# giesselmann/STRique

Measured on AMD Instinct MI355X. Metric: reads/s for STRique 'count' on 50 kb r9.4 signals, higher is better.
Workload: dtype f32

## Files before the change

strique_amd/csrc/screen_kernels.hip:

```cpp
#include "strq_opt.h"
#include <hip/hip_runtime.h>
#include <stdint.h>
#include <stdlib.h>
#include <cmath>
#include "screen_kernels.h"
#include "screen_lds_layout.h"
#include "screen_levels_layout.h"

namespace strq {

namespace {

constexpr int R = STRQ_SCREEN_R, S = STRQ_SCREEN_S, SEG = STRQ_SCREEN_SEG;
constexpr int G = 2, C = 3;
static_assert(R == 14 && S == 6, "class expansion below is written for 14 rows per lane, 6 samples per class");

__device__ __forceinline__ int dpp_shr1(int v, int fill)
{
    return __builtin_amdgcn_update_dpp(fill, v, 0x138, 0xF, 0xF, false);
}
__device__ __forceinline__ int dpp_shr1_open(int v)
{
    return __builtin_amdgcn_mov_dpp(v, 0x138, 0xF, 0xF, true);
}
// ... 181 lines not shown
                    lc.lo2[c] = lo * 2; lc.hi2[c] = (lo + w1) * 2;
                    lc.off[c] = (off - lo) * 2;
                } else {
                    lc.lo2[c] = 0; lc.hi2[c] = 0; lc.off[c] = zero_idx * 2;
                }
            }
            pm[0] = 0;
#pragma unroll
            for (int x = 1; x < 3; ++x) {
                const uint64_t b = __ballot(phase >= S - x * G);
                const uint32_t lo = __builtin_amdgcn_readfirstlane((int)(uint32_t)b), hi = __builtin_amdgcn_readfirstlane((int)(uint32_t)(b >> 32));
                pm[x] = ((uint64_t)hi << 32) | lo;
            }
        }
        const int lM = (tk.m - 1) / R;
        Screen f{ldsb, lc, pm, lane, tk.n, sp.hh};
        {
#pragma unroll
            for (int r = 0; r < R; ++r) f.T[r] = STRQ_SCREEN_BIAS;
            f.SbotA = STRQ_SCREEN_BIAS; f.upS = STRQ_SCREEN_BIAS;
            f.potB = STRQ_SCREEN_BIAS - 2 * lane * sp.hh;
            f.cmax = STRQ_SCREEN_BIAS;
        }
        const int nsteps = (tk.n + 1) / 2 + 63;
        int qcur = load_chunk(tk, 0, lane);
        f.prime(qcur);
        for (int t0s = 0; t0s < nsteps; t0s += 64) {
            const int qnext = load_chunk(tk, t0s / 64 + 1, lane);
            const bool full = (t0s >= 63) && (2 * (t0s + 64) <= tk.n);
            const int send = nsteps - t0s < 64 ? nsteps - t0s : 64;
            if (full) {
                for (int s = 0; s < 63; ++s) f.template step<false>(t0s + s + 1, qcur, s + 1);
                f.template step<false>(t0s + 64, qnext, 0);
            } else {
                for (int s = 0; s < send; ++s) {
                    const int qsrc = s == 63 ? qnext : qcur, snext = (s + 1) & 63;
                    f.template step<true>(t0s + s + 1, qsrc, snext);
                }
            }
            const int cm = __builtin_amdgcn_readlane(f.cmax, lM) - STRQ_SCREEN_BIAS;
            if (lane == 0) tk.out[t0s / 64] = cm;
            f.cmax = STRQ_SCREEN_BIAS;
            qcur = qnext;
        }
    }
}

namespace {

constexpr int CPL = STRQ_SCREEN2_CPL, LPF = STRQ_SCREEN2_LPF, LB = STRQ_SCREEN2_LANE_B;

struct Lane2Const { int lo2[CPL], hi2[CPL], off[CPL]; };

template <int RPC, int CMG, int LAYOUT>
struct Screen2 {
    static constexpr int R2 = RPC * CPL;
    static constexpr bool LEVELS = LAYOUT == STRQ_SCREEN_LDS_LEVELS;
    static_assert(CMG == 1 || CMG == 2 || CMG == 4, "groups must divide the 64 steps of a chunk");
    const char* lds;
    const Lane2Const& lc;
    const uint64_t top_mask;
    const int lane, n, hh;
    int T[R2], SbotA, upS, potB, cmax;
    int gpot, gmax;
    int qq;
    int scA[CPL], scB[CPL];

    template <bool HI>
    __device__ __forceinline__ int column(int qpair) const
    {
        if constexpr (LEVELS) return HI ? mad3_hi16(qpair, lc.off[0]) : mad3_lo16(qpair, lc.off[0]);
        else return HI ? (int)((unsigned)qpair >> 16) : (qpair & 0xffff);
    }
    __device__ __forceinline__ int score(int q2, int c) const
    {
        if constexpr (LEVELS) return *reinterpret_cast<const uint8_t*>(lds + q2 + screen_levels::class_offset(c));
        else return *reinterpret_cast<const uint16_t*>(lds + med3i(q2, lc.lo2[c], lc.hi2[c]) + lc.off[c]);
    }
    __device__ __forceinline__ void prime(int qcur)
    {
        qq = __builtin_amdgcn_update_dpp(__builtin_amdgcn_readlane(qcur, 0), 0, 0x138, 0xF, 0xF, false);
        const int qa = column<false>(qq), qb = column<true>(qq);
#pragma unroll
        for (int c = 0; c < CPL; ++c) { scA[c] = score(qa, c); scB[c] = score(qb, c); }
    }

    template <bool PRED>
    __device__ __forceinline__ void step(int t, int qsrc, int snext, bool gfirst = true, bool glast = true)
    {
        const int qn = __builtin_amdgcn_update_dpp(__builtin_amdgcn_readlane(qsrc, snext), qq, 0x138, 0xF, 0xF, false);
        const int qa = column<false>(qn), qb = column<true>(qn);
        const int potA = add_uniform(potB, hh), potBn = add_uniform(potA, hh);
        const int upA = sel_mask(dpp_shr1_open(SbotA), potA, top_mask);
        const int upB = sel_mask(dpp_shr1_open(T[R2 - 1]), potBn, top_mask);
        constexpr bool GROUPED = !PRED && CMG > 1;
        if (GROUPED && gfirst) gpot = potA;
        bool act = true, okB = true;
        if constexpr (PRED) { const int jB = 2 * (t - lane), jA = jB - 1; act = (jA >= 1) && (jA <= n); okB = jB <= n; }
        int ta_prev = upA, ta_prev2 = upS;
        int tb_prev2 = upB;
#pragma unroll
        for (int c = 0; c < CPL; ++c) {
            if (act) {
#pragma unroll
                for (int r = RPC * c; r < RPC * c + RPC; ++r) {
                    const int diagA = r == 0 ? upS : T[r - 1];
                    const int ta = max3i(diagA + scA[c], T[r], ta_prev);
                    if (r > 0) {
                        const int tb = max3i(ta_prev2 + scB[(r - 1) / RPC], ta_prev, tb_prev2);
                        T[r - 1] = tb; tb_prev2 = tb;
                    }
                    ta_prev2 = ta_prev; ta_prev = ta;
                }
                if (c == CPL - 1) {
                    const int tb = max3i(ta_prev2 + scB[c], ta_prev, tb_prev2);
                    T[R2 - 1] = tb;
                    SbotA = ta_prev;
                    upS = upB;
                    if constexpr (GROUPED) {
                        if (glast) { const int d = tb - gpot; gmax = d > gmax ? d : gmax; }
                    } else {
                        const int cA = ta_prev - potA + STRQ_SCREEN_BIAS, cB = okB ? tb - potBn + STRQ_SCREEN_BIAS : cA;
                        cmax = max3i(cmax, cA, cB);
                    }
                }
            }
            scA[c] = score(qa, c);
            if (c > 0) scB[c - 1] = score(qb, c - 1);
            if (c == CPL - 1) scB[c] = score(qb, c);
        }
        potB = potBn;
        qq = qn;
    }
};

template <int SHIFT, bool LEVELS>
__device__ __forceinline__ int load_chunk2(const Screen2Task& tk, int chunk, int lane, int lvl0, int lvl1)
{
    const int idx = (chunk * 64 + lane) * 2;
    int a = 0, b = 0;
    if (idx < tk.n) a = tk.levels[idx];
    if (idx + 1 < tk.n) b = tk.levels[idx + 1];
    if constexpr (LEVELS) return screen_levels::scaled_level(a, lvl0, lvl1) | (screen_levels::scaled_level(b, lvl0, lvl1) << 16);
    else return (a << SHIFT) | (b << (SHIFT + 16));
}

template <int RPC, int CMG, int LAYOUT, int SEGW>
__device__ __forceinline__ void screen2_body(const Screen2Task* __restrict__ tasks, int n_groups, int* __restrict__ queue, const ScreenParams& sp, int lds_rows)
{
    constexpr int R2 = RPC * CPL, MERGE = S / RPC;
    constexpr bool LANES = LAYOUT == STRQ_SCREEN_LDS_LANES, LEVELS = LAYOUT == STRQ_SCREEN_LDS_LEVELS;
    constexpr int QSHIFT = LANES ? screen_lanes::ROW_SHIFT : 1;
    constexpr int UNIT = LEVELS ? MERGE : 1;
    static_assert(!LEVELS || (MERGE == screen_levels::MERGE && SEGW == screen_levels::SEG && CPL == screen_levels::CPL), "the level image is the coarse screen's");
    static_assert((SEGW & (SEGW - 1)) == 0, "the prologue deals rows to waves by a mask");
    static_assert(CPL == screen_lanes::CPL, "screen_lds_layout.h stacks the lane's five classes");
    extern __shared__ uint32_t lds_all[];
    __shared__ int next_group;
    const int lane = threadIdx.x & 63, wave = threadIdx.x >> 6;
    const char* ldsb = reinterpret_cast<const char*>(lds_all);
    const int f = lane >= LB ? 1 : 0, lf = lane - f * LB;
    for (;;) {
        __syncthreads();
        if (threadIdx.x == 0) next_group = atomicAdd(queue, 1);
        __syncthreads();
        const int gi = __builtin_amdgcn_readfirstlane(next_group);
        if (gi >= n_groups) break;
        const Screen2Task& t0 = tasks[(size_t)gi * SEGW];
        const int ksc = LEVELS ? sp.byte_sc : sp.sc;
        const int khh = LEVELS ? sp.hh * ksc / sp.sc : sp.hh, kcadd = LEVELS ? khh + sp.v * ksc / sp.sc : sp.cadd;
        const float scf = (float)ksc;
        Lane2Const lc;
        [[maybe_unused]] int lvl0 = 0, lvl1 = 0;
        if constexpr (LEVELS) {
            lvl0 = screen_levels::range_lo(t0.lvl); lvl1 = screen_levels::range_hi(t0.lvl);
            uint32_t desc[CPL];
            int nc = 0;
#pragma unroll
            for (int c = 0; c < CPL; ++c) {
                const int k = lf * CPL + c;
                const bool in = lf < LPF && k < t0.k[f];
                desc[c] = in ? (uint32_t)t0.band_lo[f][k] : 0u;
                nc += in ? 1 : 0;
            }
            char* dst = reinterpret_cast<char*>(lds_all) + screen_levels::slot(lane);
            const float* src = t0.table[f];
            const int rows = lvl1 - lvl0 + 1 < lds_rows ? lvl1 - lvl0 + 1 : lds_rows;
            for (int r = wave; r < rows; r += SEGW) {
                int e[CPL];
#pragma unroll
                for (int c = 0; c < CPL; ++c) {
                    e[c] = 0;
                    if (c < nc) {
                        const int v = ceil_scaled(src[screen_levels::desc_off(desc[c]) + screen_levels::band_index(desc[c], lvl0 + r)], scf) + kcadd;
                        e[c] = v < 255 ? v : 255;
                    }
                }
                char* row = dst + r * screen_levels::ROW_BYTES;
                *reinterpret_cast<uint16_t*>(row + screen_levels::class_offset(0)) = (uint16_t)(e[0] | (e[1] << 8));
                *reinterpret_cast<uint16_t*>(row + screen_levels::class_offset(2)) = (uint16_t)(e[2] | (e[3] << 8));
                *reinterpret_cast<uint16_t*>(row + screen_levels::class_offset(4)) = (uint16_t)e[4];
            }
#pragma unroll
            for (int c = 0; c < CPL; ++c) { lc.lo2[c] = 0; lc.hi2[c] = 0; lc.off[c] = screen_levels::slot(lane); }
        }
        if constexpr (LANES) {
            uint32_t desc[CPL];
            int nc = 0, rowbase[CPL];
#pragma unroll
            for (int c = 0; c < CPL; ++c) {
                const int k = lf * CPL + c;
                const bool in = lf < LPF && k < t0.k[f];
                desc[c] = in ? (uint32_t)t0.band_lo[f][k] : 0u;
                nc += in ? 1 : 0;
            }
            screen_lanes::row_bases(desc, nc, rowbase);
            char* dst = reinterpret_cast<char*>(lds_all);
            if (wave == 0) *reinterpret_cast<uint16_t*>(dst + screen_lanes::slot(lane)) = 0;
#pragma unroll
            for (int c = 0; c < CPL; ++c) {
                const screen_lanes::ClassAddr a = c < nc ? screen_lanes::class_addr(lane, rowbase[c], desc[c]) : screen_lanes::padding_addr(lane);
                lc.lo2[c] = a.lo2; lc.hi2[c] = a.hi2; lc.off[c] = a.off;
                if (c < nc) {
                    const float* src = t0.table[f] + screen_lanes::desc_off(desc[c]);
                    const int w1 = screen_lanes::desc_w1(desc[c]);
                    for (int i = (wave - rowbase[c]) & (SEGW - 1); i <= w1; i += SEGW)
                        if (rowbase[c] + i < lds_rows)
                            *reinterpret_cast<uint16_t*>(dst + screen_lanes::entry_address(lane, rowbase[c], i)) = (uint16_t)(MERGE * (ceil_scaled(src[i], scf) + sp.cadd));
                }
            }
        }
        [[maybe_unused]] int base[2], zero_idx[2];
        base[0] = 0; zero_idx[0] = (t0.tsize[0] + 1) & ~1;
        base[1] = zero_idx[0] + 2; zero_idx[1] = base[1] + ((t0.tsize[1] + 1) & ~1);
        if constexpr (!LANES && !LEVELS) {
            uint16_t* dst = reinterpret_cast<uint16_t*>(lds_all);
#pragma unroll
            for (int ff = 0; ff < 2; ++ff) {
                for (int i = threadIdx.x; i < t0.tsize[ff]; i += 64 * SEGW) dst[base[ff] + i] = (uint16_t)(MERGE * (ceil_scaled(t0.table[ff][i], scf) + sp.cadd));
                if (threadIdx.x == 0) { dst[zero_idx[ff]] = 0; dst[zero_idx[ff] + 1] = 0; }
            }
        }
        __syncthreads();
        const Screen2Task& tk = tasks[(size_t)gi * SEGW + wave];
        if (tk.n <= 0) continue;

        if constexpr (!LANES && !LEVELS) {
#pragma unroll
            for (int c = 0; c < CPL; ++c) {
                const int k = lf * CPL + c;
                if (lf < LPF && k < tk.k[f]) {
                    const uint32_t d = (uint32_t)tk.band_lo[f][k];
                    const int lo = (int)(d & 255u), w1 = (int)((d >> 8) & 255u), off = (int)(d >> 16);
                    lc.lo2[c] = lo * 2; lc.hi2[c] = (lo + w1) * 2;
                    lc.off[c] = (base[f] + off - lo) * 2;
                } else {
                    lc.lo2[c] = 0; lc.hi2[c] = 0; lc.off[c] = zero_idx[f] * 2;
                }
            }
        }
        const uint64_t top_mask = 1ull | (1ull << LB);
        const int lMa = (tk.k[0] - 1) / CPL, lMb = LB + (tk.k[1] - 1) / CPL;
        const int hh = khh / UNIT;
        Screen2<RPC, CMG, LAYOUT> s2{ldsb, lc, top_mask, lane, tk.n, hh};
        {
#pragma unroll
            for (int r = 0; r < R2; ++r) s2.T[r] = STRQ_SCREEN_BIAS;
            s2.SbotA = STRQ_SCREEN_BIAS; s2.upS = STRQ_SCREEN_BIAS;
            s2.potB = STRQ_SCREEN_BIAS - 2 * lane * hh;
            s2.cmax = STRQ_SCREEN_BIAS; s2.gpot = 0; s2.gmax = 0;
        }
        const int nsteps = (tk.n + 1) / 2 + 63;
        int qcur = load_chunk2<QSHIFT, LEVELS>(tk, 0, lane, lvl0, lvl1);
        s2.prime(qcur);
        for (int t0s = 0; t0s < nsteps; t0s += 64) {
            const int qnext = load_chunk2<QSHIFT, LEVELS>(tk, t0s / 64 + 1, lane, lvl0, lvl1);
            const bool full = (t0s >= 63) && (2 * (t0s + 64) <= tk.n);
            const int send = nsteps - t0s < 64 ? nsteps - t0s : 64;
            if (full) {
                constexpr int U = CMG > 2 ? CMG : 2;
                s2.gmax = 0;
#pragma unroll 1
                for (int s = 0; s < 64 - U; s += U) {
#pragma unroll
                    for (int u = 0; u < U; ++u) s2.template step<false>(0, qcur, s + u + 1, u % CMG == 0, u % CMG == CMG - 1);
                }
#pragma unroll
                for (int u = 0; u < U - 1; ++u) s2.template step<false>(0, qcur, 64 - U + u + 1, u % CMG == 0, u % CMG == CMG - 1);
                s2.template step<false>(0, qnext, 0, CMG == 1, true);
                if constexpr (CMG > 1) s2.cmax = s2.gmax + STRQ_SCREEN_BIAS;
            } else {
                for (int s = 0; s < send; ++s) {
                    const int qsrc = s == 63 ? qnext : qcur, snext = (s + 1) & 63;
                    s2.template step<true>(t0s + s + 1, qsrc, snext);
                }
            }
            const int cma = __builtin_amdgcn_readlane(s2.cmax, lMa) - STRQ_SCREEN_BIAS;
            const int cmb = __builtin_amdgcn_readlane(s2.cmax, lMb) - STRQ_SCREEN_BIAS;
            if (lane == 0) {
                if constexpr (LEVELS) {
                    tk.out[0][t0s / 64] = (int)(((long long)cma * UNIT * sp.sc + ksc - 1) / ksc);
                    tk.out[1][t0s / 64] = (int)(((long long)cmb * UNIT * sp.sc + ksc - 1) / ksc);
                } else { tk.out[0][t0s / 64] = cma; tk.out[1][t0s / 64] = cmb; }
            }
            s2.cmax = STRQ_SCREEN_BIAS;
            qcur = qnext;
        }
    }
}

}

size_t screen2_lds_bytes(int tsize_a, int tsize_b)
{
    return (size_t)(((tsize_a + 1) & ~1) + 2 + ((tsize_b + 1) & ~1) + 2) * 2;
}

int screen2_lanes_rows(int need_a, int need_b) { return screen_lanes::rows_bound(need_a, need_b); }
bool screen2_lanes_fit(int rows) { return screen_lanes::fits(rows); }
size_t screen2_lanes_lds_bytes(int rows) { return screen_lanes::bytes(rows); }

#ifndef STRQ_SCREEN3_CMG
#define STRQ_SCREEN3_CMG 2
#endif
#define STRQ_SCREEN2_ATTR_SEG(WPE_, SEG_) __attribute__((amdgpu_flat_work_group_size(64 * SEG_, 64 * SEG_), amdgpu_waves_per_eu(WPE_, WPE_)))
#define STRQ_SCREEN2_ATTR(WPE_) STRQ_SCREEN2_ATTR_SEG(WPE_, STRQ_SCREEN_SEG)
#define STRQ_SCREEN2_ARGS const Screen2Task* __restrict__ tasks, int n_groups, int* __restrict__ queue, ScreenParams sp, int lds_rows
__global__ void STRQ_SCREEN2_ATTR_SEG(6, STRQ_SCREEN_SEG_LEVELS) align_screen3_kernel(STRQ_SCREEN2_ARGS) { screen2_body<2, STRQ_SCREEN3_CMG, STRQ_SCREEN_LDS_LEVELS, STRQ_SCREEN_SEG_LEVELS>(tasks, n_groups, queue, sp, lds_rows); }
__global__ void STRQ_SCREEN2_ATTR(6) align_screen3_lanes_kernel(STRQ_SCREEN2_ARGS) { screen2_body<2, STRQ_SCREEN3_CMG, STRQ_SCREEN_LDS_LANES, STRQ_SCREEN_SEG>(tasks, n_groups, queue, sp, lds_rows); }
__global__ void STRQ_SCREEN2_ATTR(4) align_screen1_kernel(STRQ_SCREEN2_ARGS) { screen2_body<6, 1, STRQ_SCREEN_LDS_LANES, STRQ_SCREEN_SEG>(tasks, n_groups, queue, sp, lds_rows); }
__global__ void STRQ_SCREEN2_ATTR(6) align_screen3_rows_kernel(STRQ_SCREEN2_ARGS) { screen2_body<2, STRQ_SCREEN3_CMG, STRQ_SCREEN_LDS_ROWS, STRQ_SCREEN_SEG>(tasks, n_groups, queue, sp, lds_rows); }
__global__ void STRQ_SCREEN2_ATTR(4) align_screen1_rows_kernel(STRQ_SCREEN2_ARGS) { screen2_body<6, 1, STRQ_SCREEN_LDS_ROWS, STRQ_SCREEN_SEG>(tasks, n_groups, queue, sp, lds_rows); }
#undef STRQ_SCREEN2_ARGS

__global__ void __launch_bounds__(256)
screen_windows_kernel(const ScreenTask* __restrict__ tasks, int n_groups, ScreenParams sp,
                      const int32_t* __restrict__ bound_scaled, ScreenWindows* __restrict__ out,
                      const int32_t* __restrict__ list, const int32_t* __restrict__ theta_list)
{
    const int lane = threadIdx.x & 63;
    const int idx = blockIdx.x * (blockDim.x >> 6) + (threadIdx.x >> 6);
    if (idx >= n_groups) return;
    const int g = list ? list[idx] : idx;
    const int SEG = sp.seg;
    const ScreenTask* tg = tasks + (size_t)g * SEG;
    const int m = tg[0].m, lM = tg[0].lane_last;
    const int shift = -m * sp.v;
    int vmax = 0;
    for (int w = 0; w < SEG; ++w) {
        if (tg[w].n <= 0) continue;
        for (int c = lane; c < tg[w].n_chunks; c += 64) { const int v = tg[w].out[c]; vmax = v > vmax ? v : vmax; }
    }
#pragma unroll
    for (int d = 32; d >= 1; d >>= 1) { const int o = __shfl_xor(vmax, d, 64); vmax = o > vmax ? o : vmax; }
    ScreenWindows r;
    r.n_win = 0; r.n_cand = 0;
    for (int k = 0; k < STRQ_SCREEN_MAX_WINDOWS; ++k) { r.lo[k] = 0; r.hi[k] = 0; }
    const int drop = (sp.margin > 0 ? sp.margin : m) + 2 * sp.slack;
    int theta = theta_list ? theta_list[idx] : vmax - drop;
    if (!theta_list && sp.max_cand > 0) {
        auto count_at = [&](int t) {
            int n = 0;
            for (int w = 0; w < SEG; ++w) {
                if (tg[w].n <= 0) continue;
                for (int c = lane; c < tg[w].n_chunks; c += 64) n += tg[w].out[c] >= t;
            }
#pragma unroll
            for (int d = 32; d >= 1; d >>= 1) n += __shfl_xor(n, d, 64);
            return n;
        };
        if (count_at(theta) > sp.max_cand) {
            int lo = theta, hi = vmax;
            while (hi - lo > 1) {
                const int mid = lo + (hi - lo) / 2;
                if (count_at(mid) > sp.max_cand) lo = mid; else hi = mid;
            }
            theta = hi;
        }
    }
    r.upper_bound = (float)(vmax + shift + sp.slack) / (float)sp.sc;
    auto scan = [&](int th, bool store) -> int {
        int nw = 0, last_hi = -(1 << 30), ncand = 0;
        for (int w = 0; w < SEG; ++w) {
            if (tg[w].n <= 0) continue;
            for (int c0 = 0; c0 < tg[w].n_chunks; c0 += 64) {
                const int c1 = c0 + lane;
                const bool cand = c1 < tg[w].n_chunks && tg[w].out[c1] >= th;
                uint64_t mask = __ballot(cand);
                while (mask) {
                    const int bit = __builtin_ctzll(mask); mask &= mask - 1;
                    const int c = c0 + bit;
                    ++ncand;
                    int lo = 128 * c - 2 * lM + 1, hi = 128 * c - 2 * lM + 128;
                    if (lo < 1) lo = 1;
                    if (hi > tg[w].n) hi = tg[w].n;
                    if (hi < lo) continue;
                    lo += tg[w].col_off; hi += tg[w].col_off;
                    if (nw > 0 && lo <= last_hi + sp.merge_gap) {
                        if (hi > last_hi) last_hi = hi;
                        if (store) {
                            const int k = nw <= STRQ_SCREEN_MAX_WINDOWS ? nw - 1 : STRQ_SCREEN_MAX_WINDOWS - 1;
                            if (hi > r.hi[k]) r.hi[k] = hi;
                            if (lo < r.lo[k]) r.lo[k] = lo;
                        }
                    } else {
                        ++nw; last_hi = hi;
                        if (store) {
                            if (nw <= STRQ_SCREEN_MAX_WINDOWS) { r.lo[nw - 1] = lo; r.hi[nw - 1] = hi; }
                            else if (hi > r.hi[STRQ_SCREEN_MAX_WINDOWS - 1]) r.hi[STRQ_SCREEN_MAX_WINDOWS - 1] = hi;
                        }
                    }
                }
            }
        }
        if (store) r.n_cand = ncand;
        return nw;
    };
    if (!theta_list && sp.max_cand > 0 && scan(theta, false) > STRQ_SCREEN_MAX_WINDOWS) {
        int lo = theta, hi = vmax;
        while (hi - lo > 1) {
            const int mid = lo + (hi - lo) / 2;
            if (scan(mid, false) > STRQ_SCREEN_MAX_WINDOWS) lo = mid; else hi = mid;
        }
        theta = hi;
    }
    {
        const double lb = (double)(theta + shift + sp.slack) / (double)sp.sc;
        float lbf = (float)lb;
        if ((double)lbf < lb) {
            int32_t bits = __float_as_int(lbf);
            bits = lbf > 0.0f ? bits + 1 : (lbf < 0.0f ? bits - 1 : 1);
            lbf = __int_as_float(bits);
        }
        r.lower_bound = lbf;
    }
    const bool ok = theta + shift > 0 && theta + shift > bound_scaled[g];
    if (ok) {
        int nw = scan(theta, true);
        if (nw > STRQ_SCREEN_MAX_WINDOWS) nw = STRQ_SCREEN_MAX_WINDOWS;
        for (int a = 1; a < nw; ++a)
            for (int b = a; b > 0 && r.lo[b] < r.lo[b - 1]; --b) {
                const int tl = r.lo[b], th = r.hi[b]; r.lo[b] = r.lo[b - 1]; r.hi[b] = r.hi[b - 1]; r.lo[b - 1] = tl; r.hi[b - 1] = th;
            }
        int kept = nw > 0 ? 1 : 0;
        for (int a = 1; a < nw; ++a) {
            if (r.lo[a] <= r.hi[kept - 1] + 1) { if (r.hi[a] > r.hi[kept - 1]) r.hi[kept - 1] = r.hi[a]; }
            else { r.lo[kept] = r.lo[a]; r.hi[kept] = r.hi[a]; ++kept; }
        }
        for (int a = kept; a < STRQ_SCREEN_MAX_WINDOWS; ++a) { r.lo[a] = 0; r.hi[a] = 0; }
        r.n_win = kept;
    }
    if (lane == 0) out[idx] = r;
}

int screen_plan(const AlignParams& p, int samples, int max_n, ScreenParams* sp)
{
    if (strq::opt("STRQ_NO_SCREEN")) return 0;
    if (samples != S) return 0;
    if (!(p.open_h == p.ext_h && p.open_v == p.ext_v)) return 0;
    if (!(p.dist_min >= 0.0f) || !(p.ext_h < 0.0f) || !(p.ext_v < 0.0f) || !(p.dist_offset > 0.0f) || !(p.dist_min <= p.dist_offset)) return 0;
    for (int sc = 1024; sc >= 16; sc >>= 1) {
        const double hh = -(double)p.ext_h * sc, v = -(double)p.ext_v * sc, smax = std::ceil((double)p.dist_offset * sc);
        if (hh != (double)(long)hh || v != (double)(long)v) continue;
        if (hh < 1 || smax + v + hh > 65000.0) continue;
        const double top = 64.0 * R * (smax + v) + ((double)max_n + 256.0) * hh + smax + v + hh + (double)STRQ_SCREEN_BIAS;
        if (top > 2.0e9) continue;
        sp->sc = sc; sp->hh = (int)hh; sp->v = (int)v; sp->cadd = (int)(hh + v);
        {
            const double rows = 64.0 * R, maxval = rows * (double)p.dist_offset;
            double p2 = 1.0; while (p2 < maxval) p2 *= 2.0;
            const double adds = rows * (1.0 + (double)p.dist_offset / -(double)p.ext_h);
            const double e = adds * p2 / 16777216.0;
            if (!(e < 1.0e4)) continue;
            sp->slack = ((int)std::ceil(e) + 1) * sc;
        }
        sp->merge_gap = 3072; sp->margin = 0; sp->max_cand = 0; sp->seg = STRQ_SCREEN_SEG; sp->byte_sc = 0;
        return 1;
    }
    return 0;
}

int screen2_plan(const AlignParams& p, int samples, int max_n, int merge, ScreenParams* sp)
{
    if (merge != 1 && merge != 3) return 0;
    if (!screen_plan(p, samples, max_n, sp)) return 0;
    while (sp->sc >= 16) {
        const double smax = std::ceil((double)p.dist_offset * sp->sc);
        if ((double)merge * (smax + sp->cadd) <= 65000.0) return 1;
        if ((sp->hh & 1) || (sp->v & 1)) return 0;
        sp->slack = (sp->slack / sp->sc) * (sp->sc / 2);
        sp->sc /= 2; sp->hh /= 2; sp->v /= 2; sp->cadd = sp->hh + sp->v;
    }
    return 0;
}

int screen2_levels_plan(const AlignParams& p, int samples, int max_n, int merge, ScreenParams* sp)
{
    if (merge != screen_levels::MERGE) return 0;
    if (!screen2_plan(p, samples, max_n, merge, sp)) return 0;
    const int bsc = screen_levels::byte_scale((double)p.ext_h, (double)p.ext_v, (double)p.dist_offset);
    if (bsc <= 0) return 0;
    const double hhb = -(double)p.ext_h * bsc;
    if ((double)(max_n + 256) * hhb / screen_levels::MERGE + 64.0 * CPL * 2 * 255.0 + (double)STRQ_SCREEN_BIAS > 2.0e9) return 0;
    sp->byte_sc = bsc; sp->seg = STRQ_SCREEN_SEG_LEVELS;
    return 1;
}

ScreenParams screen2_byte_frame(const ScreenParams& sp)
{
    ScreenParams b = sp;
    const int bsc = sp.byte_sc;
    b.hh = (int)((long long)sp.hh * bsc / sp.sc); b.v = (int)((long long)sp.v * bsc / sp.sc); b.cadd = b.hh + b.v;
    b.slack = sp.slack / sp.sc * bsc; b.sc = bsc; b.seg = STRQ_SCREEN_SEG; b.byte_sc = 0;
    return b;
}

uint32_t screen2_levels_range(uint32_t lvl_a, uint32_t lvl_b) { return screen_levels::join_ranges(lvl_a, lvl_b); }
int screen2_levels_rows(uint32_t range) { return screen_levels::rows_of(range); }
bool screen2_levels_fit(int rows) { return screen_levels::fits(rows); }
size_t screen2_levels_lds_bytes(int rows) { return screen_levels::bytes(rows); }

int launch_screen2(hipStream_t stream, const Screen2Task* tasks, int n_groups, int* queue, const ScreenParams& sp,
                   size_t lds_bytes, int groups_per_cu, int n_cu, int merge, int layout, int rows)
{
    if (n_groups <= 0) return 0;
    if (merge != 3 && merge != 1) return 2;
    const bool lanes = layout == STRQ_SCREEN_LDS_LANES, levels = layout == STRQ_SCREEN_LDS_LEVELS;
    if (!lanes && !levels && layout != STRQ_SCREEN_LDS_ROWS) return 2;
    if (lanes && (!screen_lanes::fits(rows) || lds_bytes < screen_lanes::bytes(rows))) return 2;
    if (levels) {
        if (merge != screen_levels::MERGE || !screen_levels::fits(rows) || lds_bytes < screen_levels::bytes(rows) || sp.seg != STRQ_SCREEN_SEG_LEVELS || sp.byte_sc <= 0) return 2;
        const ScreenParams b = screen2_byte_frame(sp);
        if (b.hh < screen_levels::MERGE || b.hh % screen_levels::MERGE != 0 || b.cadd > 255 || (long long)b.hh * sp.sc != (long long)sp.hh * b.sc) return 2;
    }
    if (!levels && sp.seg != SEG) return 2;
    auto kern = merge == 3 ? (levels ? align_screen3_kernel : lanes ? align_screen3_lanes_kernel : align_screen3_rows_kernel) : (lanes ? align_screen1_kernel : align_screen1_rows_kernel);
    if (merge == 1 && groups_per_cu > 4) groups_per_cu = 4;
    if (groups_per_cu > 6) groups_per_cu = 6;
    (void)hipFuncSetAttribute((const void*)kern, hipFuncAttributeMaxDynamicSharedMemorySize, (int)lds_bytes);
    hipLaunchKernelGGL(kern, dim3(groups_per_cu * n_cu), dim3(64 * sp.seg), lds_bytes, stream, tasks, n_groups, queue, sp, lanes || levels ? rows : 0);
    return hipGetLastError() == hipSuccess ? 0 : 1;
}

int launch_screen(hipStream_t stream, const ScreenTask* tasks, int n_groups, int* queue, const ScreenParams& sp,
                  size_t lds_bytes, int tables_per_cu, int n_cu)
{
    if (n_groups <= 0) return 0;
    (void)hipFuncSetAttribute((const void*)align_screen_kernel, hipFuncAttributeMaxDynamicSharedMemorySize, (int)lds_bytes);
    hipLaunchKernelGGL(align_screen_kernel, dim3(tables_per_cu * n_cu), dim3(64 * SEG), lds_bytes, stream, tasks, n_groups, queue, sp);
    return hipGetLastError() == hipSuccess ? 0 : 1;
}

int launch_screen_windows(hipStream_t stream, const ScreenTask* tasks, int n_groups, const ScreenParams& sp,
                          const int32_t* bound_scaled, ScreenWindows* out, const int32_t* list, const int32_t* theta_list)
{
    if (n_groups <= 0) return 0;
    hipLaunchKernelGGL(screen_windows_kernel, dim3((n_groups + 3) / 4), dim3(256), 0, stream, tasks, n_groups, sp, bound_scaled, out, list, theta_list);
    return hipGetLastError() == hipSuccess ? 0 : 1;
}

}
```

strique_amd/csrc/screen_levels_layout.h:

```cpp
#pragma once
#include <stddef.h>
#include <stdint.h>

#if defined(__HIPCC__) || defined(__CUDACC__)
#define STRQ_LEVELS_HD __host__ __device__ __forceinline__
#else
#define STRQ_LEVELS_HD inline
#endif

namespace strq {
namespace screen_levels {

constexpr int SUB_BYTES = 128;
constexpr int SUBS = 3;
constexpr int ROW_BYTES = SUBS * SUB_BYTES;
constexpr int Q_SHIFT = 7;
constexpr int CPL = 5;
constexpr int MERGE = 3;
constexpr int SEG = 8;
static_assert(SUB_BYTES == 1 << Q_SHIFT && 255 * SUB_BYTES < 65536, "a scaled level has to fit the 16-bit half of the level pair");

constexpr int MAX_ROWS = 183;
constexpr size_t MAX_BYTES = (size_t)MAX_ROWS * ROW_BYTES;

STRQ_LEVELS_HD int desc_lo(uint32_t d) { return (int)(d & 255u); }
STRQ_LEVELS_HD int desc_w1(uint32_t d) { return (int)((d >> 8) & 255u); }
STRQ_LEVELS_HD int desc_off(uint32_t d) { return (int)(d >> 16); }

STRQ_LEVELS_HD uint32_t pack_range(int lvl0, int lvl1) { return (uint32_t)lvl0 | ((uint32_t)lvl1 << 8); }
STRQ_LEVELS_HD int range_lo(uint32_t r) { return (int)(r & 255u); }
STRQ_LEVELS_HD int range_hi(uint32_t r) { return (int)((r >> 8) & 255u); }
STRQ_LEVELS_HD uint32_t join_ranges(uint32_t a, uint32_t b)
{
    const int lo = range_lo(a) < range_lo(b) ? range_lo(a) : range_lo(b), hi = range_hi(a) > range_hi(b) ? range_hi(a) : range_hi(b);
    return pack_range(lo, hi < lo ? lo : hi);
}
STRQ_LEVELS_HD int rows_of(uint32_t r) { return range_hi(r) - range_lo(r) + 1; }

STRQ_LEVELS_HD int slot(int lane) { return (lane & 31) * 4 + (lane >> 5) * 2; }
STRQ_LEVELS_HD int class_offset(int c) { return (c >> 1) * SUB_BYTES + (c & 1); }

STRQ_LEVELS_HD int scaled_level(int level, int lvl0, int lvl1)
{
    const int l = level < lvl0 ? lvl0 : (level > lvl1 ? lvl1 : level);
    return (l - lvl0) << Q_SHIFT;
}
STRQ_LEVELS_HD int column_address(int scaled, int lane) { return scaled * SUBS + slot(lane); }
STRQ_LEVELS_HD int address(int lane, int c, int level, int lvl0, int lvl1) { return column_address(scaled_level(level, lvl0, lvl1), lane) + class_offset(c); }
STRQ_LEVELS_HD int band_index(uint32_t desc, int level)
{
    const int lo = desc_lo(desc), w1 = desc_w1(desc);
    return level < lo ? 0 : (level > lo + w1 ? w1 : level - lo);
}

STRQ_LEVELS_HD size_t bytes(int rows) { return (size_t)rows * ROW_BYTES; }
STRQ_LEVELS_HD bool fits(int rows) { return rows >= 1 && rows <= MAX_ROWS; }

inline int byte_scale(double ext_h, double ext_v, double dist_offset)
{
    for (int sc = 255; sc >= 1; --sc) {
        const double hh = -ext_h * sc, v = -ext_v * sc;
        if (hh != (double)(long)hh || v != (double)(long)v || hh < MERGE) continue;
        if ((long)hh % MERGE != 0) continue;
        const double top = dist_offset * sc;
        const long smax = (long)top + ((double)(long)top < top ? 1 : 0);
        if ((double)smax + hh + v > 255.0) continue;
        return sc;
    }
    return 0;
}

}
}
```

strique_amd/csrc/strq_align_api.hip:

```cpp
#include <hip/hip_runtime.h>
#include <algorithm>
#include <cmath>
#include <climits>
#include <cstring>
#include <cstdlib>
#include <time.h>
#include <unistd.h>
#include <map>
#include <mutex>
#include <string>
#include <tuple>
#include <numeric>
#include <vector>
#include "../../include/strique_hip.h"
#include "strq_ctx.h"
#include "align_kernels.h"
#include "lut_kernels.h"
#include "align_generic.h"

using namespace strq;

#define STRQ_DBG(...) do { if (strq::opt("STRQ_DEBUG")) { fprintf(stderr, "[strq] " __VA_ARGS__); fprintf(stderr, "\n"); fflush(stderr); } } while (0)

namespace strq {
// ... 391 lines not shown
        const uint32_t lvl = F == 2 ? screen2_levels_range((uint32_t)p.info[p.J0[a[0]]].lvl, (uint32_t)p.info[p.J0[a[1]]].lvl) : 0u;
        if (F == 2) j.levels_rows = std::max(j.levels_rows, screen2_levels_rows(lvl));
        for (int f = 0; f < F; ++f)
            j.bound[(size_t)g * F + f] = used <= 1 ? INT32_MIN / 2 : (ov_s >= ov_worst ? 0 : (int32_t)std::ceil((double)align_segment_min_score(p.c->ap, in.m[a[f]], ov_s) * sp.sc));
        for (int w = 0; w < SSEG; ++w) {
            Screen2Task t; std::memset(&t, 0, sizeof(t));
            t.levels = in.d_levels + in.read_off[in.read[a[0]]] + pc[w].col_off;
            t.n = pc[w].n; t.col_off = pc[w].col_off; t.lvl = lvl;
            t.n_chunks = pc[w].n > 0 ? (align_num_steps(pc[w].n) + 63) / 64 : 0;
            for (int f = 0; f < F; ++f) {
                const LutJob& job = p.jobs[p.J0[a[f]]];
                t.table[f] = job.table; t.band_lo[f] = job.band_lo; t.tsize[f] = p.info[p.J0[a[f]]].total; t.k[f] = in.k[a[f]];
                ScreenTask v; std::memset(&v, 0, sizeof(v));
                v.n = pc[w].n; v.m = in.m[a[f]]; v.k = in.k[a[f]]; v.col_off = pc[w].col_off; v.n_chunks = t.n_chunks;
                if (F == 2) v.lane_last = f * STRQ_SCREEN2_LANE_B + (in.k[a[f]] - 1) / STRQ_SCREEN2_CPL;
                else { v.levels = t.levels; v.table = t.table[0]; v.band_lo = t.band_lo[0]; v.tsize = t.tsize[0]; v.lane_last = (v.m - 1) / STRQ_SCREEN_R; }
                j.out_off[((size_t)g * F + f) * SSEG + w] = j.out_words; j.out_words += (size_t)t.n_chunks;
                j.views[((size_t)g * F + f) * SSEG + w] = v;
            }
            if (pc[w].n > 0) j.steps += align_num_steps(pc[w].n);
            if (F == 2) j.t2[(size_t)g * SSEG + w] = t;
        }
    }
}

static int run_screen(CorePlan& p, ScreenJob& j, const ScreenParams& sp, const ScreenRules& r)
{
    const int SSEG = sp.seg;
    strq_ctx* c = p.c; const AlignCoreIn& in = p.in;
    hipStream_t st = p.st;
    const int nv = (int)j.al.size();
    int layout = 0, image_rows = 0;
    if (j.flanks == 2) {
        const char* e = strq::opt("STRQ_SCREEN_LDS");
        layout = STRQ_SCREEN_LDS_ROWS;
        if (j.layout == STRQ_SCREEN_LDS_LEVELS) { layout = STRQ_SCREEN_LDS_LEVELS; image_rows = j.levels_rows; j.lds_bytes = screen2_levels_lds_bytes(image_rows); }
        else if (!(e && std::strcmp(e, "rows") == 0) && screen2_lanes_fit(j.lanes_rows)) { layout = STRQ_SCREEN_LDS_LANES; image_rows = j.lanes_rows; j.lds_bytes = screen2_lanes_lds_bytes(image_rows); }
    }
    if (j.lds_bytes > 160 * 1024 - 64) { c->err = r.lds_err; return STRQ_ERR_UNSUPPORTED; }
    const int groups = std::max(1, std::min(r.groups_per_cu, (int)((160 * 1024 - 64) / j.lds_bytes)));
    auto aligned = [](size_t bytes) { return (bytes + 255) & ~(size_t)255; };
    const size_t t2_bytes = aligned(j.t2.size() * sizeof(Screen2Task)), task_bytes = aligned(j.views.size() * sizeof(ScreenTask));
    const size_t bound_bytes = aligned((size_t)nv * 4), win_bytes = aligned((size_t)nv * sizeof(ScreenWindows));
    STRQ_HIP(c, c->screen.reserve(t2_bytes + task_bytes + bound_bytes + win_bytes + j.out_words * 4 + 256));
    char* base = c->screen.as<char>();
    Screen2Task* d_t2 = reinterpret_cast<Screen2Task*>(base);
    ScreenTask* d_st = reinterpret_cast<ScreenTask*>(base + t2_bytes);
    int32_t* d_bound = reinterpret_cast<int32_t*>(base + t2_bytes + task_bytes);
    ScreenWindows* d_win = reinterpret_cast<ScreenWindows*>(base + t2_bytes + task_bytes + bound_bytes);
    int32_t* d_out = reinterpret_cast<int32_t*>(base + t2_bytes + task_bytes + bound_bytes + win_bytes);
    for (size_t x = 0; x < j.views.size(); ++x) j.views[x].out = d_out + j.out_off[x];
    if (j.flanks == 2)
        for (int v = 0; v < nv; ++v) for (int w = 0; w < SSEG; ++w) j.t2[(size_t)(v / 2) * SSEG + w].out[v % 2] = j.views[(size_t)v * SSEG + w].out;
    if (j.flanks == 2) STRQ_HIP(c, hipMemcpyAsync(d_t2, j.t2.data(), j.t2.size() * sizeof(Screen2Task), hipMemcpyHostToDevice, st));
    STRQ_HIP(c, hipMemcpyAsync(d_st, j.views.data(), j.views.size() * sizeof(ScreenTask), hipMemcpyHostToDevice, st));
    STRQ_HIP(c, hipMemcpyAsync(d_bound, j.bound.data(), (size_t)nv * 4, hipMemcpyHostToDevice, st));
    STRQ_HIP(c, hipEventRecord(c->ev[5], st));
    int* queue = c->queue.as<int>() + STRQ_QUEUE_FIRST - 1;
    if (j.flanks == 2) {
        if (launch_screen2(st, d_t2, nv / 2, queue, sp, j.lds_bytes, groups, c->n_cu, r.merge, layout, image_rows)) { c->err = "coarse screen launch failed"; return STRQ_ERR_DEVICE; }
    } else {
        if (launch_screen(st, d_st, nv, queue, sp, j.lds_bytes, groups, c->n_cu)) { c->err = "screen launch failed"; return STRQ_ERR_DEVICE; }
    }
    STRQ_HIP(c, hipEventRecord(c->ev[6], st));
    if (launch_screen_windows(st, d_st, nv, sp, d_bound, d_win)) { c->err = "screen windows launch failed"; return STRQ_ERR_DEVICE; }
    std::vector<ScreenWindows> hw((size_t)nv);
    STRQ_HIP(c, hipMemcpyAsync(hw.data(), d_win, hw.size() * sizeof(ScreenWindows), hipMemcpyDeviceToHost, st));
    STRQ_HIP(c, hipStreamSynchronize(st));
    c->screen_ran = true; c->screen_mode_last = r.merge > 1 ? 2 : 1; c->coarse_merge_last = r.merge;
    c->screen_lds_last = layout; c->screen_byte_sc_last = layout == STRQ_SCREEN_LDS_LEVELS ? sp.byte_sc : 0;
    if (const char* path = strq::opt("STRQ_SCREEN_DUMP")) {
        std::vector<int32_t> ho(j.out_words);
        STRQ_HIP(c, hipMemcpy(ho.data(), d_out, j.out_words * 4, hipMemcpyDeviceToHost));
        if (FILE* fp = fopen(path, "wb")) {
            const int32_t hdr[8] = {nv, sp.sc, sp.hh, sp.v, j.flanks, SSEG, sp.slack, r.merge};
            fwrite(hdr, 4, 8, fp);
            for (int v = 0; v < nv; ++v) {
                const int32_t gh[4] = {j.al[v], j.al[v], j.bound[v], j.views[(size_t)v * SSEG].lane_last};
                fwrite(gh, 4, 4, fp);
                for (int w = 0; w < SSEG; ++w) {
                    const ScreenTask& t = j.views[(size_t)v * SSEG + w];
                    const int32_t th[4] = {t.col_off, t.n, t.m, t.n_chunks};
                    fwrite(th, 4, 4, fp);
                    fwrite(ho.data() + (t.out - d_out), 4, (size_t)t.n_chunks, fp);
                }
                fwrite(&hw[(size_t)v], sizeof(ScreenWindows), 1, fp);
            }
            fclose(fp);
        }
    }
    if (const char* e = strq::opt("STRQ_SCREEN_TEST_RAISE")) {
        const float up = (float)atof(e);
        for (auto& w : hw) w.lower_bound += up;
    }
    int windowed = 0, heavy = 0, below_bound = 0; double cols = 0, all = 0;
    for (int v = 0; v < nv; ++v) {
        const int al = j.al[v];
        const ScreenWindows& w = hw[(size_t)v];
        c->screen_stats[1] += 1; c->screen_stats[7] += w.n_cand;
        double mine = in.n[al];
        if (w.n_win > 0) {
            p.wins[al] = w; c->screen_stats[2] += 1; ++windowed; mine = 0;
            for (int k = 0; k < w.n_win; ++k) { c->screen_stats[4] += w.hi[k] - w.lo[k] + 1; mine += w.hi[k] - w.lo[k] + 1 + 4096; }
        } else {
            c->screen_stats[3] += 1;
            if (w.n_cand == 0) { ++below_bound; if (r.below_bound_free) mine = 0; }
        }
        all += in.n[al]; cols += mine; heavy += mine > 4 * 32768.0;
    }
    if (r.count_untaken) c->screen_stats[3] += p.nb - nv;
    c->screen_stats[5] += j.steps; c->screen_stats[6] = sp.sc;
    if (j.flanks == 2) {
        p.screen2_ran = true;
        p.d_st2 = d_st; p.d_bound2 = d_bound; p.sp2 = sp;
        for (int v = 0; v < nv; ++v) p.g2_of[j.al[v]] = v;
        p.coarse_cols = cols; p.coarse_all = all;
    }
    if (r.judge && nv >= 64) {
        if (below_bound * 10 > nv && !p.ov_fixed) c->score_fracs.clear();
        else if (windowed < 0.9 * (nv - (p.ov_fixed ? 0 : below_bound)) || cols > r.max_cols * all || (long)heavy * 100 > 2L * nv) pause_after_fail(*r.pause, *r.fail);
        else *r.fail = 0;
    }
    STRQ_DBG("screen (%d flanks per wave, merge %d, LDS layout %d, %d image rows, %d pieces): %d alignments, scale %d, margin %.0f, %d groups per CU, LDS %zu bytes: %d with windows (%d below the cold-start bound), %.2f %% of the columns, %d heavy -> pause %d",
             j.flanks, r.merge, layout, image_rows, SSEG, nv, sp.sc, (double)sp.margin / sp.sc, groups, j.lds_bytes, windowed, below_bound, 100.0 * cols / std::max(1.0, all), heavy, *r.pause);
    return STRQ_OK;
}

static int screen_two_flank(CorePlan& p, int merge, int max_n)
{
    strq_ctx* c = p.c; const AlignCoreIn& in = p.in;
    const int nb = p.nb;
    ScreenParams sp;
    if (!screen2_plan(c->ap, p.S, max_n, merge, &sp)) return STRQ_OK;
    const bool fine_rules = merge == 1;
    int min_n = fine_rules ? 65536 : 28672, groups = 6;
    if (const char* e = strq::opt("STRQ_SCREEN_MIN_N")) min_n = atoi(e);
    if (const char* e = strq::opt("STRQ_SCREEN2_GROUPS")) { const int v = atoi(e); if (v >= 1 && v <= 8) groups = v; }
    std::map<int, std::vector<int>> by_read;
    for (int i = 0; i < nb; ++i)
        if (in.NS[i] == 1 && p.NJ[i] == 1 && in.n[i] >= min_n && screen2_flank_ok(in.m[i], in.k[i])) by_read[in.read[i]].push_back(i);
    std::vector<std::pair<int, int>> pairs;
    for (auto& kv : by_read) {
        const std::vector<int>& v = kv.second;
        if (v.size() == 2) { pairs.emplace_back(v[0], v[1]); continue; }
        for (size_t x = 0; x + 1 < v.size(); ++x)
            if (!(v[x] & 1) && v[x + 1] == v[x] + 1) { pairs.emplace_back(v[x], v[x + 1]); ++x; }
    }
    std::stable_sort(pairs.begin(), pairs.end(), [&](const std::pair<int, int>& x, const std::pair<int, int>& y) { return in.n[x.first] > in.n[y.first]; });
    const int ngr = (int)pairs.size();
    if (ngr == 0 || 2 * ngr < (nb * 9) / 10) return STRQ_OK;
    bool levels = false;
    if (merge == 3) {
        const char* e = strq::opt("STRQ_SCREEN_LDS");
        ScreenParams spb;
        if (screen2_levels_plan(c->ap, p.S, max_n, merge, &spb)) {
            levels = !e || std::strcmp(e, "levels") == 0;
            for (size_t x = 0; levels && x < pairs.size(); ++x)
                levels = screen2_levels_fit(screen2_levels_rows(screen2_levels_range((uint32_t)p.info[p.J0[pairs[x].first]].lvl, (uint32_t)p.info[p.J0[pairs[x].second]].lvl)));
            if (levels && !e) {
                double extra = 0, all = 0; long used = 0;
                for (const auto& pr : pairs) {
                    const int m_big = std::max(in.m[pr.first], in.m[pr.second]);
                    const int ov_s = overlap_for(p, m_big, align_segment_overlap(c->ap, m_big), 16);
                    Piece pc[STRQ_SCREEN_SEG_MAX];
                    const int u8 = cut(in.n[pr.first], STRQ_SCREEN_SEG_LEVELS, ov_s, pc), u4 = cut(in.n[pr.first], STRQ_SCREEN_SEG, ov_s, pc);
                    extra += (double)(u8 - u4) * ov_s; all += in.n[pr.first]; used += u8;
                }
                levels = extra <= 0.10 * all && used * 10 >= 9L * STRQ_SCREEN_SEG_LEVELS * (long)pairs.size();
            }
            if (levels) sp = spb;
            else if (strq::opt("STRQ_SCREEN2_BYTE_SCALE")) sp = screen2_byte_frame(spb);
        }
    }
    sp.margin = (int32_t)std::lround((double)c->coarse_margin * (merge == 3 ? 1.3 : 1.0) * sp.sc);
    if (const char* e = strq::opt("STRQ_SCREEN2_MARGIN")) sp.margin = (int32_t)std::lround(atof(e) * sp.sc);
    sp.max_cand = 8;
    if (const char* e = strq::opt("STRQ_SCREEN2_MAX_CAND")) sp.max_cand = atoi(e);
    if (fine_rules) { sp.margin = 0; sp.max_cand = 0; }
    ScreenJob j;
    j.flanks = 2;
    for (const auto& pr : pairs) { j.al.push_back(pr.first); j.al.push_back(pr.second); }
    j.layout = levels ? STRQ_SCREEN_LDS_LEVELS : 0;
    screen_tasks(p, sp, j);
    ScreenRules r;
    r.merge = merge; r.groups_per_cu = groups;
    r.lds_err = "score tables do not fit LDS (coarse screen)";
    r.below_bound_free = !p.ov_fixed; r.count_untaken = true;
    if (fine_rules) { r.judge = !p.scr_forced; r.max_cols = 0.15; r.pause = &c->screen_pause; r.fail = &c->screen_fail; }
    else { r.judge = !p.mode_coarse && !p.scr_forced; r.max_cols = 0.30; r.pause = &c->coarse_pause; r.fail = &c->coarse_fail; }
    return run_screen(p, j, sp, r);
}

static int screen_one_flank(CorePlan& p, const ScreenParams& sp)
{
    strq_ctx* c = p.c; const AlignCoreIn& in = p.in;
    int min_n = 65536;
    if (const char* e = strq::opt("STRQ_SCREEN_MIN_N")) min_n = atoi(e);
    std::vector<int> sel;
    for (int i = 0; i < p.nb; ++i)
        if (in.NS[i] == 1 && p.NJ[i] == 1 && in.n[i] >= min_n && screen_flank_ok(in.m[i]) && in.k[i] * p.S == in.m[i]) sel.push_back(i);
    std::stable_sort(sel.begin(), sel.end(), [&](int x, int y) { return in.n[x] > in.n[y]; });
    if (sel.empty()) return STRQ_OK;
    ScreenJob j;
    j.al = sel;
    screen_tasks(p, sp, j);
    ScreenRules r;
    r.merge = 0; r.groups_per_cu = 6;
    r.lds_err = "score table does not fit LDS (screen)";
    r.below_bound_free = false; r.count_untaken = false;
    r.judge = true; r.max_cols = 0.10; r.pause = &c->screen_pause; r.fail = &c->screen_fail;
    return run_screen(p, j, sp, r);
}

static int run_screens(CorePlan& p)
{
    strq_ctx* c = p.c; const AlignCoreIn& in = p.in;
    const int nb = p.nb;
    p.wins.resize(nb);
    c->screen_ran = false;
    STRQ_HIP(c, hipEventRecord(c->ev[2], p.st));
    int max_n = 0;
    for (int i = 0; i < nb; ++i) max_n = std::max(max_n, in.n[i]);
    c->screen_mode_last = 0;
    const int coarse_merge = 3;
    p.g2_of.assign(nb, -1);
    for (int attempt = 0; attempt < 2 && !p.screen2_ran; ++attempt) {
        int merge = coarse_merge;
        if (attempt == 0) {
            if (!p.collapsed || p.mode_fine || strq::opt("STRQ_NO_SCREEN")) continue;
            if (c->coarse_pause > 0 && !p.mode_coarse && !p.scr_forced) { --c->coarse_pause; continue; }
        } else {
            if (!p.collapsed || strq::opt("STRQ_NO_SCREEN") || (c->screen_pause > 0 && !p.scr_forced)) continue;
            merge = 1;
        }
        const int rc = screen_two_flank(p, merge, max_n);
        if (rc) return rc;
    }
    if (p.screen2_ran) return STRQ_OK;
    if (p.collapsed && c->screen_pause > 0 && !p.scr_forced) {
        --c->screen_pause; c->screen_stats[3] += nb;
        return STRQ_OK;
    }
    ScreenParams sp;
    if (p.collapsed && screen_plan(c->ap, p.S, max_n, &sp)) return screen_one_flank(p, sp);
    return STRQ_OK;
}

static int plan_launches(CorePlan& p)
{
    strq_ctx* c = p.c; const AlignCoreIn& in = p.in; AlignCoreOut& out = p.out;
    const int nb = p.nb;
    std::vector<ScreenWindows>& wins = p.wins;
    static const double rate[5][2] = {{0, 0}, {1.017, 0.941}, {0.79, 0.862}, {0.85, 0.85}, {0.69, 0.80}};
    p.packed.assign(nb, 0); p.overlap.assign(nb, 0); p.segs_of.assign(nb, 1);
    std::vector<char> segmentable(nb, 0);
    const bool force_pack = strq::opt("STRQ_PACK") != nullptr;
    int class_count[5] = {0, 0, 0, 0, 0};
    for (int i = 0; i < nb; ++i) {
        segmentable[i] = p.collapsed && in.NS[i] == 1;
        p.overlap[i] = segmentable[i] ? align_segment_overlap(c->ap, in.m[i]) : 0;
        const bool can_pack = p.allow_pack && in.NS[i] == 1 && p.info[p.J0[i]].packed && p.info[p.J0[i]].n_hard == 0;
        int best_s = 1, best_p = can_pack ? 1 : 0;
        if (segmentable[i]) {
            const double l = overlap_for(p, in.m[i], p.overlap[i]);
            double best_cost = 0;
            for (int sgs : {1, 2, 3, 4}) {
                if (p.seg_want ? sgs != p.seg_want : sgs == 3) continue;
                if (sgs > 1 && !p.seg_want && (l <= 0 || in.n[i] < (sgs + 1) * l)) continue;
                for (int pk = 0; pk < 2; ++pk) {
                    if ((pk && !can_pack) || (force_pack && can_pack && !pk)) continue;
                    const double cost = (in.n[i] + (sgs - 1) * l) * rate[sgs][pk];
                    if (best_cost == 0 || cost < best_cost) { best_cost = cost; best_s = sgs; best_p = pk; }
                }
            }
        }
        if (wins[i].n_win > 0) {
            ScreenWindows& w = wins[i];
            while (w.n_win < STRQ_SCREEN_MAX_WINDOWS) {
                int widest = 0;
                for (int k2 = 1; k2 < w.n_win; ++k2) if (w.hi[k2] - w.lo[k2] > w.hi[widest] - w.lo[widest]) widest = k2;
                if (w.hi[widest] - w.lo[widest] < 16384) break;
                const int mid = w.lo[widest] + (w.hi[widest] - w.lo[widest]) / 2;
                for (int k2 = w.n_win; k2 > widest + 1; --k2) { w.lo[k2] = w.lo[k2 - 1]; w.hi[k2] = w.hi[k2 - 1]; }
                w.lo[widest + 1] = mid + 1; w.hi[widest + 1] = w.hi[widest]; w.hi[widest] = mid;
                ++w.n_win;
            }
            const int nw = w.n_win;
            best_s = p.seg_want >= nw ? p.seg_want : (nw <= 2 ? nw : 4); best_p = 0;
        }
        p.segs_of[i] = best_s; p.packed[i] = (char)best_p;
        ++class_count[best_s];
    }
    std::vector<int>& segs_of = p.segs_of;
    if (!p.seg_want && !c->screen_ran) {
        int few = 2 * c->n_cu;
        if (const char* e = strq::opt("STRQ_CLASS_MIN")) few = atoi(e);
        if (class_count[4] && class_count[4] < few) { for (int i = 0; i < nb; ++i) if (segs_of[i] == 4) { segs_of[i] = 2; if (wins[i].n_win > 2) wins[i].n_win = 0; } class_count[2] += class_count[4]; class_count[4] = 0; }
        if (class_count[2] && class_count[2] < few && class_count[1]) { for (int i = 0; i < nb; ++i) if (segs_of[i] == 2) { segs_of[i] = 1; if (wins[i].n_win > 1) wins[i].n_win = 0; } class_count[1] += class_count[2]; class_count[2] = 0; }
    }
    std::map<std::tuple<int, int, int, int, int>, std::vector<int>> groups;
    for (int i = 0; i < nb; ++i) {
        const int w = tables_for(p, p.packed[i] ? packed_dwords(p.tab_total[i]) : p.tab_total[i], segs_of[i]);
        if (w < 1) { c->err = "score table does not fit LDS"; return STRQ_ERR_UNSUPPORTED; }
        groups[std::make_tuple(in.R[i], in.NS[i], -segs_of[i], -w, p.packed[i] ? 0 : 1)].push_back(i);
    }
    const int min_rounds = 4;
    for (auto it = groups.begin(); it != groups.end();) {
        auto nx = std::next(it);
        const int w = -std::get<3>(it->first);
        const bool same_kind = nx != groups.end() && std::get<0>(nx->first) == std::get<0>(it->first) && std::get<1>(nx->first) == std::get<1>(it->first)
                               && std::get<2>(nx->first) == std::get<2>(it->first)
                               && !(std::get<4>(it->first) == 1 && std::get<4>(nx->first) == 0);
        if (same_kind && (long)it->second.size() < (long)min_rounds * w * c->n_cu) {
            nx->second.insert(nx->second.end(), it->second.begin(), it->second.end());
            it = groups.erase(it);
        } else ++it;
    }
    out.order.clear(); out.order.reserve(nb);
    for (auto& g : groups) {
        auto& v = g.second;
        auto work = [&](int x) {
            if (wins[x].n_win <= 0) return (long)in.n[x];
            long w = 0;
            for (int k = 0; k < wins[x].n_win; ++k) w += wins[x].hi[k] - wins[x].lo[k] + 1 + 4096;
            return w;
        };
        std::stable_sort(v.begin(), v.end(), [&](int x, int y) { return work(x) > work(y); });
        const int NS = std::get<1>(g.first);
        const int pk = std::get<4>(g.first) == 0;
// ... 952 lines not shown
```

Before: 27020.

## Add merge-6 coarse screen kernel over byte level image with one row per class

Adds a coarser screen variant that merges six samples per class (one row per class) using the levels LDS layout, with a byte scale chosen for that merge factor. By default it is picked when the levels plan allows it and there are more than twice as many groups as CUs. Otherwise it falls back to merge 3. With the coarser screen the candidate cap rises to 16. The intent is to cut coarse-screen DP work roughly in half. The cost is a looser bound, which may pass more candidates on to the fine stage.

```diff
diff --git a/strique_amd/csrc/screen_kernels.hip b/strique_amd/csrc/screen_kernels.hip
--- a/strique_amd/csrc/screen_kernels.hip
+++ b/strique_amd/csrc/screen_kernels.hip
@@ -357,7 +357,7 @@
     constexpr bool LANES = LAYOUT == STRQ_SCREEN_LDS_LANES, LEVELS = LAYOUT == STRQ_SCREEN_LDS_LEVELS;
     constexpr int QSHIFT = LANES ? screen_lanes::ROW_SHIFT : 1;
     constexpr int UNIT = LEVELS ? MERGE : 1;
-    static_assert(!LEVELS || (MERGE == screen_levels::MERGE && SEGW == screen_levels::SEG && CPL == screen_levels::CPL), "the level image is the coarse screen's");
+    static_assert(!LEVELS || (screen_levels::merge_ok(MERGE) && SEGW == screen_levels::SEG && CPL == screen_levels::CPL), "the level image is the coarse screen's");
     static_assert((SEGW & (SEGW - 1)) == 0, "the prologue deals rows to waves by a mask");
     static_assert(CPL == screen_lanes::CPL, "screen_lds_layout.h stacks the lane's five classes");
     extern __shared__ uint32_t lds_all[];
@@ -532,6 +532,7 @@
 #define STRQ_SCREEN2_ATTR(WPE_) STRQ_SCREEN2_ATTR_SEG(WPE_, STRQ_SCREEN_SEG)
 #define STRQ_SCREEN2_ARGS const Screen2Task* __restrict__ tasks, int n_groups, int* __restrict__ queue, ScreenParams sp, int lds_rows
 __global__ void STRQ_SCREEN2_ATTR_SEG(6, STRQ_SCREEN_SEG_LEVELS) align_screen3_kernel(STRQ_SCREEN2_ARGS) { screen2_body<2, STRQ_SCREEN3_CMG, STRQ_SCREEN_LDS_LEVELS, STRQ_SCREEN_SEG_LEVELS>(tasks, n_groups, queue, sp, lds_rows); }
+__global__ void STRQ_SCREEN2_ATTR_SEG(6, STRQ_SCREEN_SEG_LEVELS) align_screen6_kernel(STRQ_SCREEN2_ARGS) { screen2_body<1, STRQ_SCREEN3_CMG, STRQ_SCREEN_LDS_LEVELS, STRQ_SCREEN_SEG_LEVELS>(tasks, n_groups, queue, sp, lds_rows); }
 __global__ void STRQ_SCREEN2_ATTR(6) align_screen3_lanes_kernel(STRQ_SCREEN2_ARGS) { screen2_body<2, STRQ_SCREEN3_CMG, STRQ_SCREEN_LDS_LANES, STRQ_SCREEN_SEG>(tasks, n_groups, queue, sp, lds_rows); }
 __global__ void STRQ_SCREEN2_ATTR(4) align_screen1_kernel(STRQ_SCREEN2_ARGS) { screen2_body<6, 1, STRQ_SCREEN_LDS_LANES, STRQ_SCREEN_SEG>(tasks, n_groups, queue, sp, lds_rows); }
 __global__ void STRQ_SCREEN2_ATTR(6) align_screen3_rows_kernel(STRQ_SCREEN2_ARGS) { screen2_body<2, STRQ_SCREEN3_CMG, STRQ_SCREEN_LDS_ROWS, STRQ_SCREEN_SEG>(tasks, n_groups, queue, sp, lds_rows); }
@@ -701,12 +702,12 @@
 
 int screen2_levels_plan(const AlignParams& p, int samples, int max_n, int merge, ScreenParams* sp)
 {
-    if (merge != screen_levels::MERGE) return 0;
-    if (!screen2_plan(p, samples, max_n, merge, sp)) return 0;
-    const int bsc = screen_levels::byte_scale((double)p.ext_h, (double)p.ext_v, (double)p.dist_offset);
+    if (!screen_levels::merge_ok(merge)) return 0;
+    if (!screen2_plan(p, samples, max_n, screen_levels::MERGE, sp)) return 0;
+    const int bsc = screen_levels::byte_scale((double)p.ext_h, (double)p.ext_v, (double)p.dist_offset, merge);
     if (bsc <= 0) return 0;
     const double hhb = -(double)p.ext_h * bsc;
-    if ((double)(max_n + 256) * hhb / screen_levels::MERGE + 64.0 * CPL * 2 * 255.0 + (double)STRQ_SCREEN_BIAS > 2.0e9) return 0;
+    if ((double)(max_n + 256) * hhb / merge + 64.0 * CPL * 2 * 255.0 + (double)STRQ_SCREEN_BIAS > 2.0e9) return 0;
     sp->byte_sc = bsc; sp->seg = STRQ_SCREEN_SEG_LEVELS;
     return 1;
 }
@@ -729,17 +730,18 @@
                    size_t lds_bytes, int groups_per_cu, int n_cu, int merge, int layout, int rows)
 {
     if (n_groups <= 0) return 0;
-    if (merge != 3 && merge != 1) return 2;
+    if (merge != 3 && merge != 1 && merge != 6) return 2;
     const bool lanes = layout == STRQ_SCREEN_LDS_LANES, levels = layout == STRQ_SCREEN_LDS_LEVELS;
     if (!lanes && !levels && layout != STRQ_SCREEN_LDS_ROWS) return 2;
     if (lanes && (!screen_lanes::fits(rows) || lds_bytes < screen_lanes::bytes(rows))) return 2;
+    if (merge == 6 && !levels) return 2;
     if (levels) {
-        if (merge != screen_levels::MERGE || !screen_levels::fits(rows) || lds_bytes < screen_levels::bytes(rows) || sp.seg != STRQ_SCREEN_SEG_LEVELS || sp.byte_sc <= 0) return 2;
+        if (!screen_levels::merge_ok(merge) || !screen_levels::fits(rows) || lds_bytes < screen_levels::bytes(rows) || sp.seg != STRQ_SCREEN_SEG_LEVELS || sp.byte_sc <= 0) return 2;
         const ScreenParams b = screen2_byte_frame(sp);
-        if (b.hh < screen_levels::MERGE || b.hh % screen_levels::MERGE != 0 || b.cadd > 255 || (long long)b.hh * sp.sc != (long long)sp.hh * b.sc) return 2;
+        if (b.hh < merge || b.hh % merge != 0 || b.cadd > 255 || (long long)b.hh * sp.sc != (long long)sp.hh * b.sc) return 2;
     }
     if (!levels && sp.seg != SEG) return 2;
-    auto kern = merge == 3 ? (levels ? align_screen3_kernel : lanes ? align_screen3_lanes_kernel : align_screen3_rows_kernel) : (lanes ? align_screen1_kernel : align_screen1_rows_kernel);
+    auto kern = merge == 6 ? align_screen6_kernel : merge == 3 ? (levels ? align_screen3_kernel : lanes ? align_screen3_lanes_kernel : align_screen3_rows_kernel) : (lanes ? align_screen1_kernel : align_screen1_rows_kernel);
     if (merge == 1 && groups_per_cu > 4) groups_per_cu = 4;
     if (groups_per_cu > 6) groups_per_cu = 6;
     (void)hipFuncSetAttribute((const void*)kern, hipFuncAttributeMaxDynamicSharedMemorySize, (int)lds_bytes);
diff --git a/strique_amd/csrc/screen_levels_layout.h b/strique_amd/csrc/screen_levels_layout.h
--- a/strique_amd/csrc/screen_levels_layout.h
+++ b/strique_amd/csrc/screen_levels_layout.h
@@ -56,12 +56,14 @@
 STRQ_LEVELS_HD size_t bytes(int rows) { return (size_t)rows * ROW_BYTES; }
 STRQ_LEVELS_HD bool fits(int rows) { return rows >= 1 && rows <= MAX_ROWS; }
 
-inline int byte_scale(double ext_h, double ext_v, double dist_offset)
+constexpr int MERGE_CLASS = 6;
+constexpr STRQ_LEVELS_HD bool merge_ok(int merge) { return merge == MERGE || merge == MERGE_CLASS; }
+inline int byte_scale(double ext_h, double ext_v, double dist_offset, int merge = MERGE)
 {
     for (int sc = 255; sc >= 1; --sc) {
         const double hh = -ext_h * sc, v = -ext_v * sc;
-        if (hh != (double)(long)hh || v != (double)(long)v || hh < MERGE) continue;
-        if ((long)hh % MERGE != 0) continue;
+        if (hh != (double)(long)hh || v != (double)(long)v || hh < merge) continue;
+        if ((long)hh % merge != 0) continue;
         const double top = dist_offset * sc;
         const long smax = (long)top + ((double)(long)top < top ? 1 : 0);
         if ((double)smax + hh + v > 255.0) continue;
diff --git a/strique_amd/csrc/strq_align_api.hip b/strique_amd/csrc/strq_align_api.hip
--- a/strique_amd/csrc/strq_align_api.hip
+++ b/strique_amd/csrc/strq_align_api.hip
@@ -567,8 +567,13 @@
     bool levels = false;
     if (merge == 3) {
         const char* e = strq::opt("STRQ_SCREEN_LDS");
+        int rows_per = e ? 3 : 6;
+        if (ngr <= 2 * c->n_cu) rows_per = 3;
+        if (const char* mg = strq::opt("STRQ_SCREEN2_MERGE")) { const int v = atoi(mg); if (v == 3 || v == 6) rows_per = v; }
         ScreenParams spb;
-        if (screen2_levels_plan(c->ap, p.S, max_n, merge, &spb)) {
+        bool plan = screen2_levels_plan(c->ap, p.S, max_n, rows_per, &spb) != 0;
+        if (!plan && rows_per == 6) { rows_per = 3; plan = screen2_levels_plan(c->ap, p.S, max_n, rows_per, &spb) != 0; }
+        if (plan) {
             levels = !e || std::strcmp(e, "levels") == 0;
             for (size_t x = 0; levels && x < pairs.size(); ++x)
                 levels = screen2_levels_fit(screen2_levels_rows(screen2_levels_range((uint32_t)p.info[p.J0[pairs[x].first]].lvl, (uint32_t)p.info[p.J0[pairs[x].second]].lvl)));
@@ -583,13 +588,14 @@
                 }
                 levels = extra <= 0.10 * all && used * 10 >= 9L * STRQ_SCREEN_SEG_LEVELS * (long)pairs.size();
             }
-            if (levels) sp = spb;
-            else if (strq::opt("STRQ_SCREEN2_BYTE_SCALE")) sp = screen2_byte_frame(spb);
-        }
-    }
-    sp.margin = (int32_t)std::lround((double)c->coarse_margin * (merge == 3 ? 1.3 : 1.0) * sp.sc);
+            if (levels) { sp = spb; merge = rows_per; }
+            else if (strq::opt("STRQ_SCREEN2_BYTE_SCALE") && screen2_levels_plan(c->ap, p.S, max_n, 3, &spb)) sp = screen2_byte_frame(spb);
+        }
+    }
+    sp.margin = (int32_t)std::lround((double)c->coarse_margin * (fine_rules ? 1.0 : 1.3) * sp.sc);
     if (const char* e = strq::opt("STRQ_SCREEN2_MARGIN")) sp.margin = (int32_t)std::lround(atof(e) * sp.sc);
     sp.max_cand = 8;
+    if (merge == 6) sp.max_cand = 16;
     if (const char* e = strq::opt("STRQ_SCREEN2_MAX_CAND")) sp.max_cand = atoi(e);
     if (fine_rules) { sp.margin = 0; sp.max_cand = 0; }
     ScreenJob j;
```

New measurement: 29460, median of 6. 9.0% higher.
